# DCASE-REPO/DESED_task

Measured on AMD Instinct MI355X. Metric: 10s-clips/sec CRNN mean-teacher train @batch48, higher is better.
Workload: dtype f32 (fp32 storage and accumulation; the dense contractions of the wide layers run as split-bf16 MFMA, 3 bf16 products per fp32 product, fp32-level accuracy; everything else exact f32)

## Files before the change

### desed_task_amd/csrc/sed_common.h

```cpp
#pragma once

#ifdef SED_EMU
#include "hip_emu.h"
#else
#include <hip/hip_runtime.h>
#define SED_DYN_SMEM(name) extern __shared__ __attribute__((aligned(16))) char name[]
#define SED_LAUNCH(kern, grid, block, smem, stream, ...) \
    hipLaunchKernelGGL(kern, grid, block, smem, stream, __VA_ARGS__)
typedef float f32x16 __attribute__((ext_vector_type(16)));
typedef float f32x4 __attribute__((ext_vector_type(4)));
typedef short s16x8 __attribute__((ext_vector_type(8)));
#endif

#include <stdint.h>

#define SED_API extern "C" __attribute__((visibility("default")))

#define SED_MAX_SMEM(kern, bytes) \
    (void)hipFuncSetAttribute((const void*)(kern), hipFuncAttributeMaxDynamicSharedMemorySize, (int)(bytes))

__global__ __launch_bounds__(256) static void sed_zero4_kernel(float* p0, int n0, float* p1, int n1, float* p2, int n2, float* p3, int n3) {
    const int i = blockIdx.x * 256 + threadIdx.x;
    if (i < n0) p0[i] = 0.f;
    if (i < n1) p1[i] = 0.f;
    if (i < n2) p2[i] = 0.f;
    if (i < n3) p3[i] = 0.f;
}
static inline void sed_zero4(hipStream_t s, float* p0, int n0, float* p1, int n1, float* p2, int n2, float* p3, int n3) {
    int n = n0 > n1 ? n0 : n1;
    n = n > n2 ? n : n2;
    n = n > n3 ? n : n3;
    if (n <= 0) return;
    SED_LAUNCH(sed_zero4_kernel, dim3((n + 255) / 256), dim3(256), 0, s, p0, n0, p1, n1, p2, n2, p3, n3);
}

#define SED_OK 0
#define SED_ERR_ARG (-1)
#define SED_ERR_LAUNCH (-2)
#define SED_ERR_UNSUPPORTED (-3)

enum { SED_TUNE_GLU_GRID_CAP = 0, SED_TUNE_GLU_BWD128_SPLIT = 1, SED_TUNE_CONVB_CK = 2, SED_TUNE_CONVB_MP = 3, SED_TUNE_B0_NOCENTER = 4, SED_TUNE_GLU_FWD128 = 5, SED_TUNE_WGRAD_NARROW = 6, SED_TUNE_WGRAD_CAP = 7,
       SED_TUNE_ATTN_VALU = 8, SED_TUNE_WGRAD_WIDE = 9, SED_TUNE_GRU_LDS_KB = 10, SED_TUNE_MEL_TAPS_MEM = 11, SED_TUNE_CONVB_TPW = 12, SED_TUNE_MEL_WAVE = 13, SED_TUNE_GEMM_NTN = 14, SED_TUNE_LINEAR_TILES = 15, SED_TUNE_COUNT = 16 };
extern int sed_tuning[SED_TUNE_COUNT];

static inline int sed_check_launch() {
    hipError_t e = hipGetLastError();
    return e == hipSuccess ? SED_OK : SED_ERR_LAUNCH;
}

__device__ __forceinline__ f32x16 mfma32(float a, float b, f32x16 c) {
#ifdef SED_EMU
    return emu_mfma_32x32x2(a, b, c);
#else
    return __builtin_amdgcn_mfma_f32_32x32x2f32(a, b, c, 0, 0, 0);
#endif
}
__device__ __forceinline__ int mfma32_row(int r, int lane) { return (r & 3) + 8 * (r >> 2) + 4 * (lane >> 5); }

__device__ __forceinline__ f32x4 mfma16(float a, float b, f32x4 c) {
#ifdef SED_EMU
    return emu_mfma_16x16x4(a, b, c);
#else
    return __builtin_amdgcn_mfma_f32_16x16x4f32(a, b, c, 0, 0, 0);
#endif
}

__device__ __forceinline__ f32x16 mfma32_bf16(s16x8 a, s16x8 b, f32x16 c) {
#ifdef SED_EMU
    return emu_mfma_32x32x16_bf16(a, b, c);
#else
    typedef __bf16 bf16x8_t __attribute__((ext_vector_type(8)));
    return __builtin_amdgcn_mfma_f32_32x32x16_bf16(__builtin_bit_cast(bf16x8_t, a), __builtin_bit_cast(bf16x8_t, b), c, 0, 0, 0);
#endif
}
__device__ __forceinline__ f32x4 mfma16_bf16(s16x8 a, s16x8 b, f32x4 c) {
#ifdef SED_EMU
    return emu_mfma_16x16x32_bf16(a, b, c);
#else
    typedef __bf16 bf16x8_t __attribute__((ext_vector_type(8)));
    return __builtin_amdgcn_mfma_f32_16x16x32_bf16(__builtin_bit_cast(bf16x8_t, a), __builtin_bit_cast(bf16x8_t, b), c, 0, 0, 0);
#endif
}
__device__ __forceinline__ unsigned short f32_to_bf16(float x) {
    unsigned u = __float_as_uint(x);
    u += 0x7FFFu + ((u >> 16) & 1u);
    return (unsigned short)(u >> 16);
}
__device__ __forceinline__ float bf16_to_f32(unsigned short h) { return __uint_as_float(((unsigned)h) << 16); }
__device__ __forceinline__ void bf16_split(float x, unsigned short& hi, unsigned short& lo) {
    hi = f32_to_bf16(x);
    lo = f32_to_bf16(x - bf16_to_f32(hi));
}

__device__ __forceinline__ float sed_sadd(float a, float b) {
#ifdef SED_EMU
    return a + b;
#else
    float r;
    asm("v_add_f32 %0, %1, %2" : "=v"(r) : "v"(a), "v"(b));
    return r;
#endif
}

__device__ __forceinline__ float sed_sfma(float a, float b, float c) {
#ifdef SED_EMU
    return fmaf(a, b, c);
#else
    float r;
    asm("v_fma_f32 %0, %1, %2, %3" : "=v"(r) : "v"(a), "v"(b), "v"(c));
    return r;
#endif
}

__device__ __forceinline__ void sed_sched_fence() {
#ifndef SED_EMU
    __builtin_amdgcn_sched_barrier(0);
#endif
}

__device__ __forceinline__ unsigned sed_alignbit(unsigned hi, unsigned lo, unsigned shift) {
#ifdef SED_EMU
    return (unsigned)(((((unsigned long long)hi) << 32) | lo) >> shift);
#else
    return __builtin_amdgcn_alignbit(hi, lo, shift);
#endif
}

template <class T_>
__device__ __forceinline__ void sed_pin(T_& x) {
#ifndef SED_EMU
    asm volatile("" : "+v"(x));
#else
    (void)x;
#endif
}
__device__ __forceinline__ void sed_opaque(int& x) {
#ifndef SED_EMU
    asm volatile("" : "+v"(x));
#else
    (void)x;
#endif
}

__device__ __forceinline__ int sed_wave_uniform(int x) {
#ifdef SED_EMU
    return x;
#else
    return __builtin_amdgcn_readfirstlane(x);
#endif
}

__device__ __forceinline__ void sed_wave_sync() {
#ifdef SED_EMU
    emu_wave_sync();
#else
    __builtin_amdgcn_fence(__ATOMIC_ACQ_REL, "wavefront");
    __builtin_amdgcn_wave_barrier();
#endif
}

__device__ __forceinline__ void bf16_split2(float a, float b, unsigned& hi, unsigned& lo) {
#ifdef SED_EMU
    unsigned short h0, l0, h1, l1;
    bf16_split(a, h0, l0);
    bf16_split(b, h1, l1);
    hi = (unsigned)h0 | ((unsigned)h1 << 16);
    lo = (unsigned)l0 | ((unsigned)l1 << 16);
#else
    typedef float f32x2_t __attribute__((ext_vector_type(2)));
    typedef __bf16 bf16x2_t __attribute__((ext_vector_type(2)));
    const f32x2_t v = {a, b};
    hi = __builtin_bit_cast(unsigned, __builtin_convertvector(v, bf16x2_t));
    const f32x2_t hf = {__uint_as_float(hi << 16), __uint_as_float(hi & 0xFFFF0000u)};
    lo = __builtin_bit_cast(unsigned, __builtin_convertvector(v - hf, bf16x2_t));
#endif
}

__device__ __forceinline__ f32x16 f32x16_zero() {
    f32x16 z;
#pragma unroll
    for (int i = 0; i < 16; ++i) z[i] = 0.f;
    return z;
}

__device__ __forceinline__ float sed_quad_xor1(float v) {
#ifdef SED_EMU
    return __shfl_xor(v, 1);
#else
    return __builtin_bit_cast(float, __builtin_amdgcn_update_dpp(0, __builtin_bit_cast(int, v), 0xB1, 0xF, 0xF, true));
#endif
}
__device__ __forceinline__ float sed_quad_xor2(float v) {
#ifdef SED_EMU
    return __shfl_xor(v, 2);
#else
    return __builtin_bit_cast(float, __builtin_amdgcn_update_dpp(0, __builtin_bit_cast(int, v), 0x4E, 0xF, 0xF, true));
#endif
}
__device__ __forceinline__ float sed_row_ror4(float v) {
#ifdef SED_EMU
    return __shfl_xor(v, 4);
#else
    return __builtin_bit_cast(float, __builtin_amdgcn_update_dpp(0, __builtin_bit_cast(int, v), 0x124, 0xF, 0xF, true));
#endif
}
__device__ __forceinline__ float sed_row_ror8(float v) {
#ifdef SED_EMU
    return __shfl_xor(v, 8);
#else
    return __builtin_bit_cast(float, __builtin_amdgcn_update_dpp(0, __builtin_bit_cast(int, v), 0x128, 0xF, 0xF, true));
#endif
}
__device__ __forceinline__ float sed_row16_max(float v) {
    v = fmaxf(v, sed_quad_xor1(v)); v = fmaxf(v, sed_quad_xor2(v));
    v = fmaxf(v, sed_row_ror4(v)); v = fmaxf(v, sed_row_ror8(v));
    return v;
}
__device__ __forceinline__ float sed_row16_sum(float v) {
    v += sed_quad_xor1(v); v += sed_quad_xor2(v);
    v += sed_row_ror4(v); v += sed_row_ror8(v);
    return v;
}
__device__ __forceinline__ float sed_half_mirror(float v) {
#ifdef SED_EMU
    return __shfl_xor(v, 7);
#else
    return __builtin_bit_cast(float, __builtin_amdgcn_update_dpp(0, __builtin_bit_cast(int, v), 0x141, 0xF, 0xF, true));
#endif
}
__device__ __forceinline__ float sed_quad_sum(float v) {
    v += sed_quad_xor1(v);
    v += sed_quad_xor2(v);
    return v;
}

__device__ __forceinline__ float wave_sum(float v) {
#pragma unroll
    for (int m = 32; m >= 1; m >>= 1) v += __shfl_xor(v, m);
    return v;
}
__device__ __forceinline__ float wave_min(float v) {
#pragma unroll
    for (int m = 32; m >= 1; m >>= 1) v = fminf(v, __shfl_xor(v, m));
    return v;
}
__device__ __forceinline__ float wave_max(float v) {
#pragma unroll
    for (int m = 32; m >= 1; m >>= 1) v = fmaxf(v, __shfl_xor(v, m));
    return v;
}

__device__ __forceinline__ uint32_t sed_mix32(uint32_t x) {
    x ^= x >> 16; x *= 0x85EBCA6Bu;
    x ^= x >> 13; x *= 0xC2B2AE35u;
    x ^= x >> 16;
    return x;
}
__device__ __forceinline__ uint32_t sed_hash(uint32_t idx, uint32_t seed) {
#ifdef SED_HASH_V1
    return sed_mix32(idx * 0x9E3779B1u + seed);
#else
    uint32_t x = idx * 0x9E3779B1u + sed_mix32(seed);
    x ^= x >> 15;
    return x * 0x2C1B3C6Du;
#endif
}

__device__ __forceinline__ void sed_specaug_draw(int* __restrict__ bounds, int b, int n, int f_param, int n_freq, int t_param,
                                                 int n_time, uint32_t seed) {
    const int i = n == 1 ? 0 : b;
    const float inv = 1.0f / 16777216.0f;
    int f0 = 0, f1 = 0, t0 = 0, t1 = 0;
    if (f_param >= 1) {
        const float value = (float)(sed_hash(4u * i + 0u, seed) >> 8) * inv * (float)f_param;
        const float min_value = (float)(sed_hash(4u * i + 1u, seed) >> 8) * inv * ((float)n_freq - value);
        f0 = (int)min_value;
        f1 = f0 + (int)value;
    }
    if (t_param >= 1) {
        const float value = (float)(sed_hash(4u * i + 2u, seed) >> 8) * inv * (float)t_param;
        const float min_value = (float)(sed_hash(4u * i + 3u, seed) >> 8) * inv * ((float)n_time - value);
        t0 = (int)min_value;
        t1 = t0 + (int)value;
    }
    bounds[4 * b] = f0; bounds[4 * b + 1] = f1; bounds[4 * b + 2] = t0; bounds[4 * b + 3] = t1;
}
__device__ __forceinline__ bool sed_keep(uint32_t idx, uint32_t seed, uint32_t threshold24) {
    return (sed_hash(idx, seed) >> 8) >= threshold24;
}

__device__ __forceinline__ float sed_sigmoid(float x) { return 1.0f / (1.0f + expf(-x)); }
__device__ __forceinline__ float sed_tanh(float x) { return 1.0f - 2.0f / (expf(2.0f * x) + 1.0f); }

__device__ __forceinline__ float sed_fast_exp(float x) {
#ifdef SED_EMU
    return exp2f(x * 1.44269504088896341f);
#else
    return __builtin_amdgcn_exp2f(x * 1.44269504088896341f);
#endif
}
__device__ __forceinline__ float sed_fast_rcp(float x) {
#ifdef SED_EMU
    return 1.0f / x;
#else
    return __builtin_amdgcn_rcpf(x);
#endif
}
__device__ __forceinline__ float sed_fast_sigmoid(float x) { return sed_fast_rcp(1.0f + sed_fast_exp(-x)); }
__device__ __forceinline__ float sed_fast_tanh(float x) { return 1.0f - 2.0f * sed_fast_rcp(sed_fast_exp(2.0f * x) + 1.0f); }

__device__ __forceinline__ void sed_wave_prio_high() {
#if !defined(SED_EMU) && !defined(SED_NO_SETPRIO)
    __builtin_amdgcn_s_setprio(3);
#endif
}

__device__ __forceinline__ void sed_mfma_prio(int on) {
#if !defined(SED_EMU) && !defined(SED_NO_SETPRIO)
    if (on) __builtin_amdgcn_s_setprio(1); else __builtin_amdgcn_s_setprio(0);
#else
    (void)on;
#endif
}

__device__ __forceinline__ void sed_dma16(const void* gptr, void* lds_wave_base) {
#ifdef SED_EMU
    memcpy((char*)lds_wave_base + 16 * emu_lane(), gptr, 16);
// ... 84 lines not shown
```

### desed_task_amd/csrc/sed_glu.hip

```cpp
#include "sed_common.h"

#ifndef GLU_ABL
#define GLU_ABL 0
#endif

template <int C, int PT, int PF>
struct GluGeom {
    static constexpr int WIN = PT * PF;
    static constexpr int CP = C + 1;
    static constexpr int NT = C >= 32 ? C / 32 : 1;
};

template <int PT, int PF>
__device__ __forceinline__ bool row_pixel(int m, int o0, int NWC, int fsh, int& o, int& t, int& f) {
    constexpr int WIN = PT * PF;
    const int q = m % WIN;
    o = o0 + m / WIN;
    const int to = o >> fsh, fo = o & ((1 << fsh) - 1);
    t = to * PT + q / PF;
    f = fo * PF + q % PF;
    return o < NWC;
}

template <int C, int PT, int PF>
// ... 1374 lines not shown
        bf16_split2(c, d, hv.y, lv.y);
        const int off = ch * RT + 4 * (rq ^ (2 * ((ch >> 4) & 7)));
        *(uint2*)(xth + off) = hv;
        *(uint2*)(xtl + off) = lv;
    };
    auto xhat4 = [&](int j, float* out4) {
        const int rqd = 8 * wm + 2 * j + hi, off = n * RT + 4 * (rqd ^ (2 * ((n >> 4) & 7)));
        const uint2 hv = *(const uint2*)(xth + off), lv = *(const uint2*)(xtl + off);
        out4[0] = bf16_pair_sum((unsigned short)(hv.x & 0xFFFFu), (unsigned short)(lv.x & 0xFFFFu));
        out4[1] = bf16_pair_sum((unsigned short)(hv.x >> 16), (unsigned short)(lv.x >> 16));
        out4[2] = bf16_pair_sum((unsigned short)(hv.y & 0xFFFFu), (unsigned short)(lv.y & 0xFFFFu));
        out4[3] = bf16_pair_sum((unsigned short)(hv.y >> 16), (unsigned short)(lv.y >> 16));
    };
    const float gsc = 0.5f * dscale;
    float g8n[8];
    auto load_g8 = [&](int tile_) {
        const int rbase = tile_ * ROWS + 32 * wm + 4 * hi;
#pragma unroll
        for (int j = 0; j < 4; ++j)
#pragma unroll
            for (int h = 0; h < 2; ++h) {
                const int rr = rbase + 8 * j + 2 * h;
                g8n[2 * j + h] = gout[(size_t)((rr < R ? rr : R - 1) / 2) * C + n];
            }
    };
    int tile = blockIdx.x;
    if (tile < ntiles) { load_tile(tile); load_g8(tile); }
    for (; tile < ntiles; tile += gridDim.x) {
        const int row0 = tile * ROWS;
        sed_opaque(lo); sed_opaque(hi); sed_opaque(n); sed_opaque(cq); sed_opaque(rq);
        normalise(ld0, row0 + 4 * rq); normalise(ld1, row0 + 4 * rq + 1); normalise(ld2, row0 + 4 * rq + 2); normalise(ld3, row0 + 4 * rq + 3);
        __syncthreads();
        store_rm(ld0, 4 * rq); store_rm(ld1, 4 * rq + 1); store_rm(ld2, 4 * rq + 2); store_rm(ld3, 4 * rq + 3);
        store_tr(ld0.x, ld1.x, ld2.x, ld3.x, 4 * cq);
        store_tr(ld0.y, ld1.y, ld2.y, ld3.y, 4 * cq + 1);
        store_tr(ld0.z, ld1.z, ld2.z, ld3.z, 4 * cq + 2);
        store_tr(ld0.w, ld1.w, ld2.w, ld3.w, 4 * cq + 3);
        __syncthreads();
        if (tile + (int)gridDim.x < ntiles) load_tile(tile + gridDim.x);
        float g8[8];
#pragma unroll
        for (int u = 0; u < 8; ++u) g8[u] = g8n[u];
        load_g8(tile + (int)gridDim.x < ntiles ? tile + gridDim.x : tile);
        f32x16 acc = f32x16_zero();
        {
            const unsigned short* ap = xh + (32 * wm + lo) * RS + 8 * hi;
#pragma unroll
            for (int ks = 0; ks < KS; ++ks) {
                const s16x8 a_hi = *(const s16x8*)(ap + 16 * ks);
                const s16x8 a_lo = *(const s16x8*)(ap + ROWS * RS + 16 * ks);
                acc = mfma32_bf16(a_lo, b1h[ks], acc);
                acc = mfma32_bf16(a_hi, b1l[ks], acc);
                acc = mfma32_bf16(a_hi, b1h[ks], acc);
            }
        }
#pragma unroll
        for (int j = 0; j < 4; ++j) {
            float dv[4], xq[4];
            xhat4(j, xq);
#pragma unroll
            for (int q = 0; q < 4; ++q) {
                const int r = 4 * j + q, m = 32 * wm + 8 * j + 4 * hi + q;
                const uint32_t e_idx = (uint32_t)(row0 + m) * (uint32_t)C + (uint32_t)n;
                float dlin = 0.f, e = 0.f;
                if (row0 + m < R) {
                    const float xn = fmaf(xq[q], gn, bn);
                    const float sg = sed_fast_sigmoid(xn);
                    const float lin = acc[r] + biasp;
                    const float g = sed_keep(e_idx, seed, thr24) ? g8[2 * j + (q >> 1)] * gsc : 0.f;
                    dlin = g * sg;
                    e = g * lin * sg * (1.0f - sg);
                }
                unsigned short hh, ll;
                bf16_split(dlin, hh, ll);
                dh[m * RS + n] = hh;
                dl[m * RS + n] = ll;
                dv[q] = dlin;
                acc[r] = e;
                a_dbg += dlin;
            }
            uint2 hv, lv;
            bf16_split2(dv[0], dv[1], hv.x, lv.x);
            bf16_split2(dv[2], dv[3], hv.y, lv.y);
            const int rqd = 8 * wm + 2 * j + hi;
            const int off = n * RT + 4 * (rqd ^ (2 * ((n >> 4) & 7)));
            *(uint2*)(dth + off) = hv;
            *(uint2*)(dtl + off) = lv;
        }
        __syncthreads();
        {
            const unsigned short* ap = dh + (32 * wm + lo) * RS + 8 * hi;
#pragma unroll
            for (int ks = 0; ks < KS; ++ks) {
                const s16x8 a_hi = *(const s16x8*)(ap + 16 * ks);
                const s16x8 a_lo = *(const s16x8*)(ap + ROWS * RS + 16 * ks);
                acc = mfma32_bf16(a_lo, b2h[ks], acc);
                acc = mfma32_bf16(a_hi, b2l[ks], acc);
                acc = mfma32_bf16(a_hi, b2h[ks], acc);
            }
        }
#pragma unroll
        for (int j = 0; j < 4; ++j) {
            float xq[4];
            xhat4(j, xq);
#pragma unroll
            for (int q = 0; q < 4; ++q) {
                const int r = 4 * j + q, m = 32 * wm + 8 * j + 4 * hi + q;
                if (row0 + m < R) {
                    const float dxn = acc[r];
                    a_dgam = fmaf(dxn, xq[q], a_dgam);
                    a_dbet += dxn;
                    dz[(size_t)(row0 + m) * C + n] = dxn * gn;
                }
            }
        }
#pragma unroll
        for (int i = 0; i < TPW; ++i) {
            const int id = NT3 >= 8 ? w * TPW + i : w % NT3, mt = id / NT, ct = id % NT;
            const int ks0 = NT3 >= 8 ? 0 : (w / NT3) * KS3;
            const int rowa = mt * 32 + lo, rowb = ct * 32 + lo;
#pragma unroll
            for (int ks = 0; ks < KS3; ++ks) {
                const int oct = 2 * (ks0 + ks) + hi;
                const int offa = rowa * RT + 8 * (oct ^ ((rowa >> 4) & 7)), offb = rowb * RT + 8 * (oct ^ ((rowb >> 4) & 7));
                const s16x8 a_hi = *(const s16x8*)(dth + offa), a_lo = *(const s16x8*)(dtl + offa);
                const s16x8 b_hi = *(const s16x8*)(xth + offb), b_lo = *(const s16x8*)(xtl + offb);
                P[i] = mfma32_bf16(a_lo, b_hi, P[i]);
                P[i] = mfma32_bf16(a_hi, b_lo, P[i]);
                P[i] = mfma32_bf16(a_hi, b_hi, P[i]);
            }
        }
    }
    float* mine = part + (size_t)blockIdx.x * (KSPLIT * C * C + WM * 3 * C);
#pragma unroll
    for (int i = 0; i < TPW; ++i) {
        const int id = NT3 >= 8 ? w * TPW + i : w % NT3, mt = id / NT, ct = id % NT, c = ct * 32 + lo;
        float* dst = mine + (NT3 >= 8 ? 0 : w / NT3) * C * C;
#pragma unroll
        for (int r = 0; r < 16; ++r) dst[(mt * 32 + mfma32_row(r, lane)) * C + c] = P[i][r];
    }
    a_dbg += __shfl_xor(a_dbg, 32); a_dgam += __shfl_xor(a_dgam, 32); a_dbet += __shfl_xor(a_dbet, 32);
    if (hi == 0) {
        float* dst = mine + KSPLIT * C * C + wm * 3 * C;
        dst[n] = a_dbg; dst[C + n] = a_dgam; dst[2 * C + n] = a_dbet;
    }
}
__global__ __launch_bounds__(512) void glu128_bwd_c_kernel(const float* __restrict__ y, const float* __restrict__ stats,
                                                           const float* __restrict__ gamma, const float* __restrict__ beta,
                                                           const float* __restrict__ Wg, const float* __restrict__ bg,
                                                           const float* __restrict__ gout, float* __restrict__ dz,
                                                           float* __restrict__ part, int B, int T, int F, uint32_t seed,
                                                           uint32_t thr24, float dscale, const unsigned* __restrict__ seed_dev) {
    if (seed_dev) seed += *seed_dev;
    constexpr int C = 128, ROWS = 64, RS = C, RT = ROWS, WS = C + 8, KS = C / 32, RB = ROWS / 16, NB = C / 16, KS3 = ROWS / 32;
    SED_DYN_SMEM(smem);
    unsigned short* xh = (unsigned short*)smem;
    unsigned short* xl = xh + ROWS * RS;
    unsigned short* xth = xl + ROWS * RS;
    unsigned short* xtl = xth + C * RT;
    unsigned short* dh = xtl + C * RT;
    unsigned short* dl = dh + ROWS * RS;
    unsigned short* dth = dl + ROWS * RS;
    unsigned short* dtl = dth + C * RT;
    const int tid = threadIdx.x, lane = tid & 63, w = tid >> 6;
    int i16 = lane & 15, g = lane >> 4;
    int n = 16 * w + i16;
    const int R = B * T * F, ntiles = (R + ROWS - 1) / ROWS;
    auto rm_off = [](int m, int k) { return m * RS + ((((k >> 3) ^ (m & 15))) << 3) + (k & 7); };
    auto tr_off = [](int ch, int row) { return ch * RT + ((((row >> 3) ^ ((ch >> 1) & 7))) << 3) + (row & 7); };
    unsigned short* wh = xh;
    unsigned short* wl = xh + 64 * WS;

    s16x8 b1h[KS], b1l[KS], b2h[KS], b2l[KS];
    float biasp = bg[n];
#pragma unroll
    for (int p = 0; p < C / 64; ++p) {
#pragma unroll
        for (int fold = 0; fold < 2; ++fold) {
            __syncthreads();
            for (int i = tid; i < 64 * (C / 4); i += 512) {
                const int row = i / (C / 4), q = i - row * (C / 4);
                float4 val = *(const float4*)(Wg + (size_t)(p * 64 + row) * C + 4 * q);
                if (fold) { val.x *= gamma[4 * q]; val.y *= gamma[4 * q + 1]; val.z *= gamma[4 * q + 2]; val.w *= gamma[4 * q + 3]; }
                uint2 hv, lv;
                bf16_split2(val.x, val.y, hv.x, lv.x);
                bf16_split2(val.z, val.w, hv.y, lv.y);
                *(uint2*)(wh + row * WS + 4 * q) = hv;
                *(uint2*)(wl + row * WS + 4 * q) = lv;
            }
            __syncthreads();
            if (!fold) {
#pragma unroll
                for (int kk = 0; kk < 2; ++kk) {
                    s16x8 fh, fl;
#pragma unroll
                    for (int e = 0; e < 8; ++e) {
                        fh[e] = (short)wh[(32 * kk + 8 * g + e) * WS + n];
                        fl[e] = (short)wl[(32 * kk + 8 * g + e) * WS + n];
                    }
                    b2h[2 * p + kk] = fh; b2l[2 * p + kk] = fl;
                }
                if (w / 4 == p) {
                    const int rown = n - p * 64;
                    float part_b = 0.f;
                    for (int k = 32 * g; k < 32 * g + 32; ++k)
                        part_b = fmaf(beta[k], bf16_pair_sum(wh[rown * WS + k], wl[rown * WS + k]), part_b);
                    part_b += __shfl_xor(part_b, 16);
                    part_b += __shfl_xor(part_b, 32);
                    biasp += part_b;
                }
            } else if (w / 4 == p) {
#pragma unroll
                for (int ks = 0; ks < KS; ++ks) {
                    b1h[ks] = *(const s16x8*)(wh + (n - p * 64) * WS + 32 * ks + 8 * g);
                    b1l[ks] = *(const s16x8*)(wl + (n - p * 64) * WS + 32 * ks + 8 * g);
                }
            }
        }
    }
    const float gn = gamma[n], bn = beta[n];
    int cq = tid % (C / 4), rq = tid / (C / 4);

    f32x4 P[NB];
#pragma unroll
    for (int i = 0; i < NB; ++i) P[i] = f32x4{0.f, 0.f, 0.f, 0.f};
    float a_dbg = 0.f, a_dgam = 0.f, a_dbet = 0.f;

    float4 ld0, ld1, ld2, ld3;
    auto load_row = [&](int row) -> float4 {
        float4 val = make_float4(0.f, 0.f, 0.f, 0.f);
        if (row < R && !(GLU_ABL & 4)) val = *(const float4*)(y + (size_t)row * C + 4 * cq);
        return val;
    };
    auto load_tile = [&](int tile) {
        const int row = tile * ROWS + 4 * rq;
        if ((tile + 1) * ROWS <= R && !(GLU_ABL & 4)) {
            const float* src = y + (size_t)row * C + 4 * cq;
            ld0 = *(const float4*)src; ld1 = *(const float4*)(src + C); ld2 = *(const float4*)(src + 2 * C); ld3 = *(const float4*)(src + 3 * C);
        } else {
            ld0 = load_row(row); ld1 = load_row(row + 1); ld2 = load_row(row + 2); ld3 = load_row(row + 3);
        }
    };
    auto normalise = [&](int tile) {
        const float4 mu = *(const float4*)(stats + 4 * cq), is = *(const float4*)(stats + C + 4 * cq);
        const int row = tile * ROWS + 4 * rq;
        auto nrm = [&](float4& v, int r) {
            const float keep = r < R ? 1.0f : 0.0f;
            v.x = (v.x - mu.x) * is.x * keep; v.y = (v.y - mu.y) * is.y * keep;
            v.z = (v.z - mu.z) * is.z * keep; v.w = (v.w - mu.w) * is.w * keep;
        };
        nrm(ld0, row); nrm(ld1, row + 1); nrm(ld2, row + 2); nrm(ld3, row + 3);
    };
    auto store_rm = [&](const float4 val, int m) {
        uint2 hv, lv;
        bf16_split2(val.x, val.y, hv.x, lv.x);
        bf16_split2(val.z, val.w, hv.y, lv.y);
        *(uint2*)(xh + rm_off(m, 4 * cq)) = hv;
        *(uint2*)(xl + rm_off(m, 4 * cq)) = lv;
    };
    auto store_tr = [&](float a, float b, float c, float d, int ch) {
        uint2 hv, lv;
        bf16_split2(a, b, hv.x, lv.x);
        bf16_split2(c, d, hv.y, lv.y);
        const int off = tr_off(ch, 4 * rq);
        *(uint2*)(xth + off) = hv;
        *(uint2*)(xtl + off) = lv;
    };
    auto xhat4 = [&](int rb, float* out4) {
        const int off = tr_off(n, 16 * rb + 4 * g);
        const uint2 hv = *(const uint2*)(xth + off), lv = *(const uint2*)(xtl + off);
        out4[0] = bf16_pair_sum((unsigned short)(hv.x & 0xFFFFu), (unsigned short)(lv.x & 0xFFFFu));
        out4[1] = bf16_pair_sum((unsigned short)(hv.x >> 16), (unsigned short)(lv.x >> 16));
        out4[2] = bf16_pair_sum((unsigned short)(hv.y & 0xFFFFu), (unsigned short)(lv.y & 0xFFFFu));
        out4[3] = bf16_pair_sum((unsigned short)(hv.y >> 16), (unsigned short)(lv.y >> 16));
    };
    auto gemm_rows = [&](const unsigned short* ph, const s16x8* bh, const s16x8* bl, f32x4* acc) {
#pragma unroll
        for (int ks = 0; ks < KS; ++ks) {
            s16x8 ah[RB], al[RB];
#pragma unroll
            for (int rb = 0; rb < RB; ++rb) {
                const unsigned short* ap = ph + rm_off(16 * rb + i16, 32 * ks + 8 * g);
                ah[rb] = *(const s16x8*)ap;
                al[rb] = *(const s16x8*)(ap + ROWS * RS);
            }
#pragma unroll
            for (int rb = 0; rb < RB; ++rb) acc[rb] = mfma16_bf16(al[rb], bh[ks], acc[rb]);
#pragma unroll
            for (int rb = 0; rb < RB; ++rb) acc[rb] = mfma16_bf16(ah[rb], bl[ks], acc[rb]);
#pragma unroll
            for (int rb = 0; rb < RB; ++rb) acc[rb] = mfma16_bf16(ah[rb], bh[ks], acc[rb]);
            sed_sched_fence();
        }
    };
    int tile = blockIdx.x;
    float g8n[2 * RB];
    auto load_g8 = [&](int tile_) {
#pragma unroll
        for (int rb = 0; rb < RB; ++rb)
#pragma unroll
            for (int h = 0; h < 2; ++h) {
                const int rr = tile_ * ROWS + 16 * rb + 4 * g + 2 * h;
                g8n[2 * rb + h] = (GLU_ABL & 4) ? 1.0f : gout[(size_t)((rr < R ? rr : 0) / 2) * C + n];
            }
    };
    if (tile < ntiles) { load_tile(tile); load_g8(tile); }
    for (; tile < ntiles; tile += gridDim.x) {
        const int row0 = tile * ROWS;
        sed_opaque(i16); sed_opaque(g); sed_opaque(n); sed_opaque(cq); sed_opaque(rq);
        normalise(tile);
        __syncthreads();
        store_rm(ld0, 4 * rq); store_rm(ld1, 4 * rq + 1); store_rm(ld2, 4 * rq + 2); store_rm(ld3, 4 * rq + 3);
        store_tr(ld0.x, ld1.x, ld2.x, ld3.x, 4 * cq);
        store_tr(ld0.y, ld1.y, ld2.y, ld3.y, 4 * cq + 1);
        store_tr(ld0.z, ld1.z, ld2.z, ld3.z, 4 * cq + 2);
        store_tr(ld0.w, ld1.w, ld2.w, ld3.w, 4 * cq + 3);
        __syncthreads();
        float g8[2 * RB];
#pragma unroll
        for (int rb = 0; rb < RB; ++rb)
#pragma unroll
            for (int h = 0; h < 2; ++h) {
                const int rr = row0 + 16 * rb + 4 * g + 2 * h;
                g8[2 * rb + h] = rr < R ? g8n[2 * rb + h] * (0.5f * dscale) : 0.f;
            }
        load_g8(tile + (int)gridDim.x < ntiles ? tile + gridDim.x : tile);
        f32x4 acc[RB];
#pragma unroll
        for (int rb = 0; rb < RB; ++rb) acc[rb] = f32x4{0.f, 0.f, 0.f, 0.f};
        if (!(GLU_ABL & 1)) gemm_rows(xh, b1h, b1l, acc);
#pragma unroll
        for (int rb = 0; rb < RB; ++rb) {
            unsigned short hh[4], ll[4];
            float xq[4];
            xhat4(rb, xq);
#pragma unroll
            for (int r = 0; r < 4; ++r) {
                const int m = 16 * rb + 4 * g + r;
                const uint32_t e_idx = (uint32_t)(row0 + m) * (uint32_t)C + (uint32_t)n;
                const float xn = fmaf(xq[r], gn, bn);
                const float sg = (GLU_ABL & 2) ? xn : sed_fast_sigmoid(xn);
                const float lin = acc[rb][r] + biasp;
                const float gq = ((GLU_ABL & 2) || sed_keep(e_idx, seed, thr24)) ? g8[2 * rb + (r >> 1)] : 0.f;
                const float dlin = gq * sg;
                const float e = gq * lin * sg * (1.0f - sg);
                bf16_split(dlin, hh[r], ll[r]);
                dh[rm_off(m, n)] = hh[r];
                dl[rm_off(m, n)] = ll[r];
                acc[rb][r] = e;
                a_dbg += dlin;
            }
            uint2 hv, lv;
            hv.x = (unsigned)hh[0] | ((unsigned)hh[1] << 16); hv.y = (unsigned)hh[2] | ((unsigned)hh[3] << 16);
            lv.x = (unsigned)ll[0] | ((unsigned)ll[1] << 16); lv.y = (unsigned)ll[2] | ((unsigned)ll[3] << 16);
            const int off = tr_off(n, 16 * rb + 4 * g);
            *(uint2*)(dth + off) = hv;
            *(uint2*)(dtl + off) = lv;
        }
        __syncthreads();
        if (!(GLU_ABL & 1)) gemm_rows(dh, b2h, b2l, acc);
        const bool full = row0 + ROWS <= R;
#pragma unroll
        for (int rb = 0; rb < RB; ++rb) {
            float xq[4];
            xhat4(rb, xq);
#pragma unroll
            for (int r = 0; r < 4; ++r) {
                const int m = 16 * rb + 4 * g + r;
                const float dxn = acc[rb][r];
                a_dgam = fmaf(dxn, xq[r], a_dgam);
                a_dbet += dxn;
                if (!(GLU_ABL & 8) && (full || row0 + m < R)) dz[(size_t)(row0 + m) * C + n] = dxn * gn;
            }
        }
        if (tile + (int)gridDim.x < ntiles) load_tile(tile + gridDim.x);
        if (!(GLU_ABL & 1)) {
            const int rowa = 16 * w + i16;
            s16x8 ah3, al3;
#pragma unroll
            for (int st = 0; st < 2 * KS3; ++st) {
                const int ks = st >> 1, c0 = 4 * (st & 1);
                if ((st & 1) == 0) {
                    const int offa = tr_off(rowa, 32 * ks + 8 * g);
                    ah3 = *(const s16x8*)(dth + offa);
                    al3 = *(const s16x8*)(dtl + offa);
                }
                s16x8 bh3[4], bl3[4];
#pragma unroll
                for (int q = 0; q < 4; ++q) {
                    const int offb = tr_off(16 * (c0 + q) + i16, 32 * ks + 8 * g);
                    bh3[q] = *(const s16x8*)(xth + offb);
                    bl3[q] = *(const s16x8*)(xtl + offb);
                }
#pragma unroll
                for (int q = 0; q < 4; ++q) P[c0 + q] = mfma16_bf16(al3, bh3[q], P[c0 + q]);
#pragma unroll
                for (int q = 0; q < 4; ++q) P[c0 + q] = mfma16_bf16(ah3, bl3[q], P[c0 + q]);
#pragma unroll
                for (int q = 0; q < 4; ++q) P[c0 + q] = mfma16_bf16(ah3, bh3[q], P[c0 + q]);
                sed_sched_fence();
            }
        }
    }
    float* mine = part + (size_t)blockIdx.x * (C * C + 3 * C);
#pragma unroll
    for (int cb = 0; cb < NB; ++cb)
#pragma unroll
        for (int r = 0; r < 4; ++r) mine[(16 * w + 4 * g + r) * C + 16 * cb + i16] = P[cb][r];
    a_dbg += __shfl_xor(a_dbg, 16); a_dgam += __shfl_xor(a_dgam, 16); a_dbet += __shfl_xor(a_dbet, 16);
    a_dbg += __shfl_xor(a_dbg, 32); a_dgam += __shfl_xor(a_dgam, 32); a_dbet += __shfl_xor(a_dbet, 32);
    if (g == 0) {
        float* dst = mine + C * C;
        dst[n] = a_dbg; dst[C + n] = a_dgam; dst[2 * C + n] = a_dbet;
    }
}
#define GBR_THREADS 1024
#define GBR_GROUPS (GBR_THREADS / 16)
__global__ __launch_bounds__(GBR_THREADS) void glu_bwd_reduce_kernel(const float* __restrict__ part, float* __restrict__ dWg,
                                                             float* __restrict__ dbg, float* __restrict__ dgamma,
                                                             float* __restrict__ dbeta, int nblk, int C, int KS, int WMS,
                                                             const float* __restrict__ gamma, const float* __restrict__ beta, int fix) {
    __shared__ float4 red[GBR_GROUPS][16];
    __shared__ float sdb[GBR_THREADS / 64];
    const int tid = threadIdx.x, col = tid & 15, grp = tid >> 4, e = blockIdx.x * 64 + 4 * col;
    const int CC = C * C, PART = KS * CC + WMS * 3 * C;
    const bool isw = e < CC;
    const int nsl = isw ? KS : WMS, sstride = isw ? CC : 3 * C;
    const size_t off = isw ? (size_t)e : (size_t)KS * CC + (e - CC);
    float4 acc = make_float4(0.f, 0.f, 0.f, 0.f);
    if (e < CC + 3 * C) {
        const int total = nblk * nsl;
#pragma unroll 4
        for (int i = grp; i < total; i += GBR_GROUPS) {
            const int b = i / nsl, k = i - b * nsl;
            const float4 v = *(const float4*)(part + (size_t)b * PART + off + (size_t)k * sstride);
            acc.x += v.x; acc.y += v.y; acc.z += v.z; acc.w += v.w;
        }
    }
    const bool need_dbn = fix && blockIdx.x * 64 < CC;
    float sacc = 0.f;
    if (need_dbn) {
        const int nrow = (blockIdx.x * 64) / C;
#pragma unroll 2
        for (int i = tid; i < nblk * WMS; i += GBR_THREADS) {
            const int b = i / WMS, k = i - b * WMS;
            sacc += part[(size_t)b * PART + (size_t)KS * CC + k * 3 * C + nrow];
        }
    }
    float4 gq = make_float4(0.f, 0.f, 0.f, 0.f), bq = gq;
    if (fix && isw && grp == 0) {
        const int c = e % C;
        gq = make_float4(gamma[c], gamma[c + 1], gamma[c + 2], gamma[c + 3]);
        bq = make_float4(beta[c], beta[c + 1], beta[c + 2], beta[c + 3]);
    }
    red[grp][col] = acc;
    if (need_dbn) {
        sacc = wave_sum(sacc);
        if ((tid & 63) == 0) sdb[tid >> 6] = sacc;
    }
    __syncthreads();
    float dbn = 0.f;
    if (need_dbn) {
#pragma unroll
        for (int w = 0; w < GBR_THREADS / 64; ++w) dbn += sdb[w];
    }
    if (grp == 0 && e < CC + 3 * C) {
#pragma unroll 8
        for (int g = 1; g < GBR_GROUPS; ++g) { const float4 v = red[g][col]; acc.x += v.x; acc.y += v.y; acc.z += v.z; acc.w += v.w; }
        if (fix && isw) {
            acc.x = fmaf(gq.x, acc.x, bq.x * dbn); acc.y = fmaf(gq.y, acc.y, bq.y * dbn);
            acc.z = fmaf(gq.z, acc.z, bq.z * dbn); acc.w = fmaf(gq.w, acc.w, bq.w * dbn);
        }
        float* dst;
        if (isw) dst = dWg + e;
        else {
            const int j2 = e - CC, which = j2 / C;
            dst = (which == 0 ? dbg : which == 1 ? dgamma : dbeta) + (j2 - which * C);
        }
        *(float4*)dst = acc;
    }
}
template <int C, bool SPLIT>
static int launch_glu_wide_bwd(const float* y, const float* stats, const float* gamma, const float* beta, const float* Wg,
                               const float* bg, const float* gout, float* dz, float* dWg, float* dbg, float* dgamma, float* dbeta,
                               float* scratch, int B, int T, int F, uint32_t seed, uint32_t thr24, float dscale, const unsigned* seed_dev, hipStream_t s) {
    constexpr int ROWS = 32 * (8 / (C / 32)), WMS = 8 / (C / 32), KS = (C / 32) * (C / 32) >= 8 ? 1 : 8 / ((C / 32) * (C / 32));
    if (!scratch) return SED_ERR_ARG;
    constexpr int SMEM = SPLIT ? 8 * (ROWS * (C + 8) + C * (ROWS + 8)) : (2 * ROWS + (C > 64 ? C : 0)) * (C + 1) * 4;
    const int ntiles = (B * T * F + ROWS - 1) / ROWS;
    const int cap = glu_grid_cap(256);
    int grid = ntiles < cap ? ntiles : cap;
    if (grid < 1) { sed_zero4(s, dWg, C * C, dbg, C, dgamma, C, dbeta, C); return SED_OK; }
    if (SPLIT && C == 128 && sed_tuning[SED_TUNE_GLU_BWD128_SPLIT] != 1) {
        constexpr int SMEM_C = 8 * 64 * 128 * 2;
        SED_MAX_SMEM(glu128_bwd_c_kernel, SMEM_C);
        SED_LAUNCH(glu128_bwd_c_kernel, dim3(grid), dim3(512), SMEM_C, s, y, stats, gamma, beta, Wg, bg, gout, dz, scratch, B, T, F,
                   seed, thr24, dscale, seed_dev);
        SED_LAUNCH(glu_bwd_reduce_kernel, dim3((C * C + 3 * C + 63) / 64), dim3(GBR_THREADS), 0, s, scratch, dWg, dbg, dgamma, dbeta, grid, C, 1, 1,
                   gamma, beta, 1);
        return sed_check_launch();
    }
    if (SPLIT) {
        SED_MAX_SMEM((glu_wide_bwd_b_kernel<C>), SMEM);
        SED_LAUNCH((glu_wide_bwd_b_kernel<C>), dim3(grid), dim3(512), SMEM, s, y, stats, gamma, beta, Wg, bg, gout, dz, scratch, B, T, F,
                   seed, thr24, dscale, seed_dev);
    } else {
        SED_MAX_SMEM((glu_wide_bwd_kernel<C>), SMEM);
        SED_LAUNCH((glu_wide_bwd_kernel<C>), dim3(grid), dim3(512), SMEM, s, y, stats, gamma, beta, Wg, bg, gout, dz, scratch, B, T, F,
                   seed, thr24, dscale, seed_dev);
    }
    SED_LAUNCH(glu_bwd_reduce_kernel, dim3((C * C + 3 * C + 63) / 64), dim3(GBR_THREADS), 0, s, scratch, dWg, dbg, dgamma, dbeta, grid, C, KS, WMS,
               gamma, beta, SPLIT ? 1 : 0);
    return sed_check_launch();
}

SED_API long long sed_glu_bwd_scratch_floats(int B, int T, int F, int C, int PT, int PF) {
    (void)B; (void)T; (void)F;
    if (PT == 1 && PF == 2 && (C == 64 || C == 128)) {
        const int nt3 = (C / 32) * (C / 32), ks = nt3 >= 8 ? 1 : 8 / nt3, wms = 8 / (C / 32);
        return 256LL * (ks * C * C + wms * 3 * C);
    }
    if (PT == 2 && PF == 2 && (C == 16 || C == 32)) return 1024LL * (C * C + 3 * C);
    return 0;
}

SED_API int sed_glu_bwd(const float* y, const float* stats, const float* gamma, const float* beta, const float* Wg,
                           const float* bg, const float* gout, float* dz, float* dWg, float* dbg, float* dgamma, float* dbeta,
                           float* scratch, int B, int T, int F, int C, int PT, int PF, unsigned seed, unsigned thr24, float dscale,
                           const unsigned* seed_dev, int split_bf16, void* stream) {
    hipStream_t s = (hipStream_t)stream;
    if (F % PF != 0) return SED_ERR_UNSUPPORTED;
    if (PT == 1 && PF == 2) {
        if (C == 128 && split_bf16 && sed_tuning[SED_TUNE_GLU_BWD128_SPLIT] != 3)
            return launch_glu_wide_bwd<128, true>(y, stats, gamma, beta, Wg, bg, gout, dz, dWg, dbg, dgamma, dbeta, scratch, B, T, F, seed, thr24, dscale, seed_dev, s);
        if (C == 64 && split_bf16) return launch_glu_wide_bwd<64, true>(y, stats, gamma, beta, Wg, bg, gout, dz, dWg, dbg, dgamma, dbeta, scratch, B, T, F, seed, thr24, dscale, seed_dev, s);
        if (C == 128) return launch_glu_wide_bwd<128, false>(y, stats, gamma, beta, Wg, bg, gout, dz, dWg, dbg, dgamma, dbeta, scratch, B, T, F, seed, thr24, dscale, seed_dev, s);
        if (C == 64) return launch_glu_wide_bwd<64, false>(y, stats, gamma, beta, Wg, bg, gout, dz, dWg, dbg, dgamma, dbeta, scratch, B, T, F, seed, thr24, dscale, seed_dev, s);
    }
    const bool lds_free32 = C == 32 && PT == 2 && PF == 2 && F % 16 == 0 && T >= 2;
    if (T % PT != 0 && !lds_free32) {
        const int tail = T % PT, rowf4 = F * C / 4;
        const long long n4 = (long long)B * tail * rowf4;
        int grid = (int)((n4 + 255) / 256);
        if (grid > 2048) grid = 2048;
        SED_LAUNCH(glu_zero_tail_kernel, dim3(grid), dim3(256), 0, s, dz, n4, T, T - tail, tail * rowf4, (long long)T * rowf4);
    }
    if ((C == 16 && PT == 2 && PF == 2 && F % 8 == 0) || (C == 32 && PT == 2 && PF == 2 && F % 16 == 0)) {
        const int nrows = B * (T / 2);
        int grid = (nrows + 3) / 4;
        const int cap = C == 32 ? glu_grid_cap(512) : 1024;
        if (grid > cap) grid = cap;
        if (grid < 1) { sed_zero4(s, dWg, C * C, dbg, C, dgamma, C, dbeta, C); return SED_OK; }
        if (!scratch) return SED_ERR_ARG;
        if (C == 16)
            SED_LAUNCH(glu16_bwd_kernel, dim3(grid), dim3(256), 0, s, y, stats, gamma, beta, Wg, bg, gout, dz, scratch, B, T, F, seed, thr24,
                       dscale, seed_dev);
        else
            SED_LAUNCH(glu32_bwd_kernel, dim3(grid), dim3(256), 0, s, y, stats, gamma, beta, Wg, bg, gout, dz, scratch, B, T, F, seed, thr24,
                       dscale, seed_dev);
        SED_LAUNCH(glu_bwd_reduce_kernel, dim3((C * C + 3 * C + 63) / 64), dim3(GBR_THREADS), 0, s, scratch, dWg, dbg, dgamma, dbeta, grid, C, 1, 1,
                   gamma, beta, 0);
        return sed_check_launch();
    }
    sed_zero4(s, dWg, C * C, dbg, C, dgamma, C, dbeta, C);
#define GLU_CASE(c, pt, pf)                                                                                              \
    if (C == c && PT == pt && PF == pf)                                                                                  \
        return launch_glu_bwd<c, pt, pf>(y, stats, gamma, beta, Wg, bg, gout, dz, dWg, dbg, dgamma, dbeta, B, T, F, seed, thr24, \
                                         dscale, seed_dev, s);
    GLU_CASE(16, 2, 2) GLU_CASE(32, 2, 2)
#undef GLU_CASE
    return SED_ERR_UNSUPPORTED;
}

template <int C>
__global__ __launch_bounds__(256) void bn_bwd_apply_kernel(const float* __restrict__ y, float* __restrict__ dz,
                                                           const float* __restrict__ stats, const float* __restrict__ gamma,
                                                           const float* __restrict__ dgamma, const float* __restrict__ dbeta,
                                                           float* __restrict__ dbias, size_t npix, float inv_count, int training) {
    constexpr int V = C / 4, RPI = 256 / V;
    const int tid = threadIdx.x, v = tid % V, r0 = tid / V;
    float mean[4], istd[4], m1[4], m2[4];
#pragma unroll
    for (int i = 0; i < 4; ++i) {
        const int c = 4 * v + i;
        mean[i] = stats[c];
        istd[i] = stats[C + c];
        m1[i] = training ? gamma[c] * dbeta[c] * inv_count : 0.f;
        m2[i] = training ? gamma[c] * dgamma[c] * inv_count : 0.f;
    }
    if (blockIdx.x == 0 && tid < C) dbias[tid] = training ? 0.f : stats[C + tid] * gamma[tid] * dbeta[tid];
    for (size_t p = (size_t)blockIdx.x * RPI + r0; p < npix; p += (size_t)gridDim.x * RPI) {
        const float4 yv = *(const float4*)(y + p * C + 4 * v);
        float4 g = *(const float4*)(dz + p * C + 4 * v);
        g.x = istd[0] * (g.x - m1[0] - (yv.x - mean[0]) * istd[0] * m2[0]);
        g.y = istd[1] * (g.y - m1[1] - (yv.y - mean[1]) * istd[1] * m2[1]);
        g.z = istd[2] * (g.z - m1[2] - (yv.z - mean[2]) * istd[2] * m2[2]);
        g.w = istd[3] * (g.w - m1[3] - (yv.w - mean[3]) * istd[3] * m2[3]);
        *(float4*)(dz + p * C + 4 * v) = g;
    }
}
SED_API int sed_bn_bwd_apply(const float* y, float* dz, const float* stats, const float* gamma, const float* dgamma,
                                const float* dbeta, float* dbias, long long npix, int C, int training, void* stream) {
    hipStream_t s = (hipStream_t)stream;
    if (npix <= 0) return SED_OK;
    const float inv = 1.0f / (float)npix;
    int grid = (int)((npix * (C / 4) + 255) / 256);
    if (grid > 4096) grid = 4096;
#define BN_CASE(c) \
    if (C == c) { SED_LAUNCH((bn_bwd_apply_kernel<c>), dim3(grid), dim3(256), 0, s, y, dz, stats, gamma, dgamma, dbeta, dbias, (size_t)npix, inv, training); return sed_check_launch(); }
    BN_CASE(16) BN_CASE(32) BN_CASE(64) BN_CASE(128)
#undef BN_CASE
    return SED_ERR_UNSUPPORTED;
}
```

Baseline: 16050.

## Double-buffer GLU128 backward tiles and use LDS transpose reads instead of transposed copies

```diff
diff --git a/desed_task_amd/csrc/sed_common.h b/desed_task_amd/csrc/sed_common.h
--- a/desed_task_amd/csrc/sed_common.h
+++ b/desed_task_amd/csrc/sed_common.h
@@ -173,6 +173,21 @@
     hi = __builtin_bit_cast(unsigned, __builtin_convertvector(v, bf16x2_t));
     const f32x2_t hf = {__uint_as_float(hi << 16), __uint_as_float(hi & 0xFFFF0000u)};
     lo = __builtin_bit_cast(unsigned, __builtin_convertvector(v - hf, bf16x2_t));
+#endif
+}
+
+template <class OFF>
+__device__ __forceinline__ uint2 sed_lds_read_tr16(const unsigned short* img, OFF off, int r0, int c0, int lane) {
+#ifdef SED_EMU
+    const int col = c0 + (lane & 15);
+    uint2 v;
+    v.x = (unsigned)img[off(r0, col)] | ((unsigned)img[off(r0 + 1, col)] << 16);
+    v.y = (unsigned)img[off(r0 + 2, col)] | ((unsigned)img[off(r0 + 3, col)] << 16);
+    return v;
+#else
+    typedef short s16x4_t __attribute__((ext_vector_type(4)));
+    const unsigned short* p = img + off(r0 + ((lane >> 2) & 3), c0 + 4 * (lane & 3));
+    return __builtin_bit_cast(uint2, __builtin_amdgcn_ds_read_tr16_b64_v4i16((__attribute__((address_space(3))) s16x4_t*)p));
 #endif
 }
 
diff --git a/desed_task_amd/csrc/sed_glu.hip b/desed_task_amd/csrc/sed_glu.hip
--- a/desed_task_amd/csrc/sed_glu.hip
+++ b/desed_task_amd/csrc/sed_glu.hip
@@ -1550,35 +1550,40 @@
                                                            float* __restrict__ part, int B, int T, int F, uint32_t seed,
                                                            uint32_t thr24, float dscale, const unsigned* __restrict__ seed_dev) {
     if (seed_dev) seed += *seed_dev;
-    constexpr int C = 128, ROWS = 64, RS = C, RT = ROWS, WS = C + 8, KS = C / 32, RB = ROWS / 16, NB = C / 16, KS3 = ROWS / 32;
+    constexpr int C = 128, ROWS = 64, WS = C + 8, KS = C / 32, RB = ROWS / 16, NB = C / 16, KS3 = ROWS / 32, PL = ROWS * C;
     SED_DYN_SMEM(smem);
-    unsigned short* xh = (unsigned short*)smem;
-    unsigned short* xl = xh + ROWS * RS;
-    unsigned short* xth = xl + ROWS * RS;
-    unsigned short* xtl = xth + C * RT;
-    unsigned short* dh = xtl + C * RT;
-    unsigned short* dl = dh + ROWS * RS;
-    unsigned short* dth = dl + ROWS * RS;
-    unsigned short* dtl = dth + C * RT;
-    const int tid = threadIdx.x, lane = tid & 63, w = tid >> 6;
-    int i16 = lane & 15, g = lane >> 4;
+    unsigned short* xbuf = (unsigned short*)smem;
+    unsigned short* dth = xbuf + 4 * PL;
+    unsigned short* dtl = dth + PL;
+    const int tid = threadIdx.x, w = tid >> 6;
+    int lane = tid & 63, i16 = lane & 15, g = lane >> 4;
     int n = 16 * w + i16;
     const int R = B * T * F, ntiles = (R + ROWS - 1) / ROWS;
-    auto rm_off = [](int m, int k) { return m * RS + ((((k >> 3) ^ (m & 15))) << 3) + (k & 7); };
-    auto tr_off = [](int ch, int row) { return ch * RT + ((((row >> 3) ^ ((ch >> 1) & 7))) << 3) + (row & 7); };
-    unsigned short* wh = xh;
-    unsigned short* wl = xh + 64 * WS;
+    auto x_off = [](int m, int k) {
+        return m * C + ((((k >> 3) ^ (int)(0xEC13B9468A75DF20ull >> (4 * (m & 15)))) & 15) << 3) + (k & 7);
+    };
+    auto d_off = [](int ch, int row) {
+        return ch * ROWS + ((((row >> 3) ^ (int)(0x4307256152163470ull >> (4 * ((ch & 3) | ((ch >> 1) & 12))))) & 7) << 3) + (row & 7);
+    };
+    unsigned short* wh = xbuf;
+    unsigned short* wl = xbuf + C * WS;
 
     s16x8 b1h[KS], b1l[KS], b2h[KS], b2l[KS];
     float biasp = bg[n];
-#pragma unroll
-    for (int p = 0; p < C / 64; ++p) {
+    {
+        float4 wv[C * (C / 4) / 512];
+#pragma unroll
+        for (int j = 0; j < C * (C / 4) / 512; ++j) {
+            const int i = tid + 512 * j, row = i / (C / 4), q = i - row * (C / 4);
+            wv[j] = *(const float4*)(Wg + (size_t)row * C + 4 * q);
+        }
 #pragma unroll
         for (int fold = 0; fold < 2; ++fold) {
-            __syncthreads();
-            for (int i = tid; i < 64 * (C / 4); i += 512) {
-                const int row = i / (C / 4), q = i - row * (C / 4);
-                float4 val = *(const float4*)(Wg + (size_t)(p * 64 + row) * C + 4 * q);
+            if (fold) __syncthreads();
+#pragma unroll
+            for (int j = 0; j < C * (C / 4) / 512; ++j) {
+                const int i = tid + 512 * j, row = i / (C / 4), q = i - row * (C / 4);
+                float4 val = wv[j];
                 if (fold) { val.x *= gamma[4 * q]; val.y *= gamma[4 * q + 1]; val.z *= gamma[4 * q + 2]; val.w *= gamma[4 * q + 3]; }
                 uint2 hv, lv;
                 bf16_split2(val.x, val.y, hv.x, lv.x);
@@ -1589,29 +1594,26 @@
             __syncthreads();
             if (!fold) {
 #pragma unroll
-                for (int kk = 0; kk < 2; ++kk) {
+                for (int ks = 0; ks < KS; ++ks) {
                     s16x8 fh, fl;
 #pragma unroll
                     for (int e = 0; e < 8; ++e) {
-                        fh[e] = (short)wh[(32 * kk + 8 * g + e) * WS + n];
-                        fl[e] = (short)wl[(32 * kk + 8 * g + e) * WS + n];
+                        fh[e] = (short)wh[(32 * ks + 8 * g + e) * WS + n];
+                        fl[e] = (short)wl[(32 * ks + 8 * g + e) * WS + n];
                     }
-                    b2h[2 * p + kk] = fh; b2l[2 * p + kk] = fl;
+                    b2h[ks] = fh; b2l[ks] = fl;
                 }
-                if (w / 4 == p) {
-                    const int rown = n - p * 64;
-                    float part_b = 0.f;
-                    for (int k = 32 * g; k < 32 * g + 32; ++k)
-                        part_b = fmaf(beta[k], bf16_pair_sum(wh[rown * WS + k], wl[rown * WS + k]), part_b);
-                    part_b += __shfl_xor(part_b, 16);
-                    part_b += __shfl_xor(part_b, 32);
-                    biasp += part_b;
-                }
-            } else if (w / 4 == p) {
+                float part_b = 0.f;
+                for (int k = 32 * g; k < 32 * g + 32; ++k)
+                    part_b = fmaf(beta[k], bf16_pair_sum(wh[n * WS + k], wl[n * WS + k]), part_b);
+                part_b += __shfl_xor(part_b, 16);
+                part_b += __shfl_xor(part_b, 32);
+                biasp += part_b;
+            } else {
 #pragma unroll
                 for (int ks = 0; ks < KS; ++ks) {
-                    b1h[ks] = *(const s16x8*)(wh + (n - p * 64) * WS + 32 * ks + 8 * g);
-                    b1l[ks] = *(const s16x8*)(wl + (n - p * 64) * WS + 32 * ks + 8 * g);
+                    b1h[ks] = *(const s16x8*)(wh + n * WS + 32 * ks + 8 * g);
+                    b1l[ks] = *(const s16x8*)(wl + n * WS + 32 * ks + 8 * g);
                 }
             }
         }
@@ -1624,7 +1626,7 @@
     for (int i = 0; i < NB; ++i) P[i] = f32x4{0.f, 0.f, 0.f, 0.f};
     float a_dbg = 0.f, a_dgam = 0.f, a_dbet = 0.f;
 
-    float4 ld0, ld1, ld2, ld3;
+    float4 ld0 = make_float4(0.f, 0.f, 0.f, 0.f), ld1 = ld0, ld2 = ld0, ld3 = ld0;
     auto load_row = [&](int row) -> float4 {
         float4 val = make_float4(0.f, 0.f, 0.f, 0.f);
         if (row < R && !(GLU_ABL & 4)) val = *(const float4*)(y + (size_t)row * C + 4 * cq);
@@ -1649,47 +1651,32 @@
         };
         nrm(ld0, row); nrm(ld1, row + 1); nrm(ld2, row + 2); nrm(ld3, row + 3);
     };
-    auto store_rm = [&](const float4 val, int m) {
+    auto store_row = [&](unsigned short* xb, const float4 val, int m) {
         uint2 hv, lv;
         bf16_split2(val.x, val.y, hv.x, lv.x);
         bf16_split2(val.z, val.w, hv.y, lv.y);
-        *(uint2*)(xh + rm_off(m, 4 * cq)) = hv;
-        *(uint2*)(xl + rm_off(m, 4 * cq)) = lv;
-    };
-    auto store_tr = [&](float a, float b, float c, float d, int ch) {
-        uint2 hv, lv;
-        bf16_split2(a, b, hv.x, lv.x);
-        bf16_split2(c, d, hv.y, lv.y);
-        const int off = tr_off(ch, 4 * rq);
-        *(uint2*)(xth + off) = hv;
-        *(uint2*)(xtl + off) = lv;
-    };
-    auto xhat4 = [&](int rb, float* out4) {
-        const int off = tr_off(n, 16 * rb + 4 * g);
-        const uint2 hv = *(const uint2*)(xth + off), lv = *(const uint2*)(xtl + off);
+        *(uint2*)(xb + x_off(m, 4 * cq)) = hv;
+        *(uint2*)(xb + PL + x_off(m, 4 * cq)) = lv;
+    };
+    auto xhat4 = [&](const unsigned short* xb, int rb, float* out4) {
+        const uint2 hv = sed_lds_read_tr16(xb, x_off, 16 * rb + 4 * g, 16 * w, lane);
+        const uint2 lv = sed_lds_read_tr16(xb + PL, x_off, 16 * rb + 4 * g, 16 * w, lane);
         out4[0] = bf16_pair_sum((unsigned short)(hv.x & 0xFFFFu), (unsigned short)(lv.x & 0xFFFFu));
         out4[1] = bf16_pair_sum((unsigned short)(hv.x >> 16), (unsigned short)(lv.x >> 16));
         out4[2] = bf16_pair_sum((unsigned short)(hv.y & 0xFFFFu), (unsigned short)(lv.y & 0xFFFFu));
         out4[3] = bf16_pair_sum((unsigned short)(hv.y >> 16), (unsigned short)(lv.y >> 16));
     };
-    auto gemm_rows = [&](const unsigned short* ph, const s16x8* bh, const s16x8* bl, f32x4* acc) {
-#pragma unroll
-        for (int ks = 0; ks < KS; ++ks) {
-            s16x8 ah[RB], al[RB];
-#pragma unroll
-            for (int rb = 0; rb < RB; ++rb) {
-                const unsigned short* ap = ph + rm_off(16 * rb + i16, 32 * ks + 8 * g);
-                ah[rb] = *(const s16x8*)ap;
-                al[rb] = *(const s16x8*)(ap + ROWS * RS);
-            }
-#pragma unroll
-            for (int rb = 0; rb < RB; ++rb) acc[rb] = mfma16_bf16(al[rb], bh[ks], acc[rb]);
-#pragma unroll
-            for (int rb = 0; rb < RB; ++rb) acc[rb] = mfma16_bf16(ah[rb], bl[ks], acc[rb]);
-#pragma unroll
-            for (int rb = 0; rb < RB; ++rb) acc[rb] = mfma16_bf16(ah[rb], bh[ks], acc[rb]);
-            sed_sched_fence();
-        }
+    auto frag8 = [](const uint2 a, const uint2 b) {
+        const uint4 v = make_uint4(a.x, a.y, b.x, b.y);
+        return __builtin_bit_cast(s16x8, v);
+    };
+    auto mfma_step = [&](const s16x8* ah, const s16x8* al, const s16x8 bh, const s16x8 bl, f32x4* acc) {
+#pragma unroll
+        for (int rb = 0; rb < RB; ++rb) acc[rb] = mfma16_bf16(al[rb], bh, acc[rb]);
+#pragma unroll
+        for (int rb = 0; rb < RB; ++rb) acc[rb] = mfma16_bf16(ah[rb], bl, acc[rb]);
+#pragma unroll
+        for (int rb = 0; rb < RB; ++rb) acc[rb] = mfma16_bf16(ah[rb], bh, acc[rb]);
     };
     int tile = blockIdx.x;
     float g8n[2 * RB];
@@ -1703,17 +1690,18 @@
             }
     };
     if (tile < ntiles) { load_tile(tile); load_g8(tile); }
-    for (; tile < ntiles; tile += gridDim.x) {
+    __syncthreads();
+    if (tile < ntiles) {
+        normalise(tile);
+        store_row(xbuf, ld0, 4 * rq); store_row(xbuf, ld1, 4 * rq + 1); store_row(xbuf, ld2, 4 * rq + 2); store_row(xbuf, ld3, 4 * rq + 3);
+        if (tile + (int)gridDim.x < ntiles) load_tile(tile + gridDim.x);
+    }
+    __syncthreads();
+    for (int buf = 0; tile < ntiles; tile += gridDim.x, buf ^= 1) {
         const int row0 = tile * ROWS;
-        sed_opaque(i16); sed_opaque(g); sed_opaque(n); sed_opaque(cq); sed_opaque(rq);
-        normalise(tile);
-        __syncthreads();
-        store_rm(ld0, 4 * rq); store_rm(ld1, 4 * rq + 1); store_rm(ld2, 4 * rq + 2); store_rm(ld3, 4 * rq + 3);
-        store_tr(ld0.x, ld1.x, ld2.x, ld3.x, 4 * cq);
-        store_tr(ld0.y, ld1.y, ld2.y, ld3.y, 4 * cq + 1);
-        store_tr(ld0.z, ld1.z, ld2.z, ld3.z, 4 * cq + 2);
-        store_tr(ld0.w, ld1.w, ld2.w, ld3.w, 4 * cq + 3);
-        __syncthreads();
+        sed_opaque(lane); sed_opaque(i16); sed_opaque(g); sed_opaque(n); sed_opaque(cq); sed_opaque(rq);
+        const unsigned short* xc = xbuf + buf * 2 * PL;
+        unsigned short* xnx = xbuf + (buf ^ 1) * 2 * PL;
         float g8[2 * RB];
 #pragma unroll
         for (int rb = 0; rb < RB; ++rb)
@@ -1726,12 +1714,25 @@
         f32x4 acc[RB];
 #pragma unroll
         for (int rb = 0; rb < RB; ++rb) acc[rb] = f32x4{0.f, 0.f, 0.f, 0.f};
-        if (!(GLU_ABL & 1)) gemm_rows(xh, b1h, b1l, acc);
+        if (!(GLU_ABL & 1)) {
+#pragma unroll
+            for (int ks = 0; ks < KS; ++ks) {
+                s16x8 ah[RB], al[RB];
+#pragma unroll
+                for (int rb = 0; rb < RB; ++rb) {
+                    const unsigned short* ap = xc + x_off(16 * rb + i16, 32 * ks + 8 * g);
+                    ah[rb] = *(const s16x8*)ap;
+                    al[rb] = *(const s16x8*)(ap + PL);
+                }
+                mfma_step(ah, al, b1h[ks], b1l[ks], acc);
+                sed_sched_fence();
+            }
+        }
 #pragma unroll
         for (int rb = 0; rb < RB; ++rb) {
             unsigned short hh[4], ll[4];
             float xq[4];
-            xhat4(rb, xq);
+            xhat4(xc, rb, xq);
 #pragma unroll
             for (int r = 0; r < 4; ++r) {
                 const int m = 16 * rb + 4 * g + r;
@@ -1743,25 +1744,41 @@
                 const float dlin = gq * sg;
                 const float e = gq * lin * sg * (1.0f - sg);
                 bf16_split(dlin, hh[r], ll[r]);
-                dh[rm_off(m, n)] = hh[r];
-                dl[rm_off(m, n)] = ll[r];
                 acc[rb][r] = e;
                 a_dbg += dlin;
             }
             uint2 hv, lv;
             hv.x = (unsigned)hh[0] | ((unsigned)hh[1] << 16); hv.y = (unsigned)hh[2] | ((unsigned)hh[3] << 16);
             lv.x = (unsigned)ll[0] | ((unsigned)ll[1] << 16); lv.y = (unsigned)ll[2] | ((unsigned)ll[3] << 16);
-            const int off = tr_off(n, 16 * rb + 4 * g);
+            const int off = d_off(n, 16 * rb + 4 * g);
             *(uint2*)(dth + off) = hv;
             *(uint2*)(dtl + off) = lv;
         }
-        __syncthreads();
-        if (!(GLU_ABL & 1)) gemm_rows(dh, b2h, b2l, acc);
+        if (!(GLU_ABL & 64)) __syncthreads();
+        normalise(tile + (int)gridDim.x);
+#pragma unroll
+        for (int ks = 0; ks < KS; ++ks) {
+            s16x8 ah[RB], al[RB];
+            int ln = lane;
+            sed_opaque(ln);
+            const int ch0 = 32 * ks + 8 * (ln >> 4);
+            if (!(GLU_ABL & 1)) {
+#pragma unroll
+                for (int rb = 0; rb < RB; ++rb) {
+                    ah[rb] = frag8(sed_lds_read_tr16(dth, d_off, ch0, 16 * rb, ln), sed_lds_read_tr16(dth, d_off, ch0 + 4, 16 * rb, ln));
+                    al[rb] = frag8(sed_lds_read_tr16(dtl, d_off, ch0, 16 * rb, ln), sed_lds_read_tr16(dtl, d_off, ch0 + 4, 16 * rb, ln));
+                }
+            }
+            store_row(xnx, ks == 0 ? ld0 : ks == 1 ? ld1 : ks == 2 ? ld2 : ld3, 4 * rq + ks);
+            if (!(GLU_ABL & 1)) mfma_step(ah, al, b2h[ks], b2l[ks], acc);
+            sed_sched_fence();
+        }
+        if (tile + 2 * (int)gridDim.x < ntiles) load_tile(tile + 2 * gridDim.x);
         const bool full = row0 + ROWS <= R;
 #pragma unroll
         for (int rb = 0; rb < RB; ++rb) {
             float xq[4];
-            xhat4(rb, xq);
+            xhat4(xc, rb, xq);
 #pragma unroll
             for (int r = 0; r < 4; ++r) {
                 const int m = 16 * rb + 4 * g + r;
@@ -1771,24 +1788,24 @@
                 if (!(GLU_ABL & 8) && (full || row0 + m < R)) dz[(size_t)(row0 + m) * C + n] = dxn * gn;
             }
         }
-        if (tile + (int)gridDim.x < ntiles) load_tile(tile + gridDim.x);
         if (!(GLU_ABL & 1)) {
-            const int rowa = 16 * w + i16;
             s16x8 ah3, al3;
 #pragma unroll
             for (int st = 0; st < 2 * KS3; ++st) {
-                const int ks = st >> 1, c0 = 4 * (st & 1);
+                int ln = lane;
+                sed_opaque(ln);
+                const int ks = st >> 1, c0 = 4 * (st & 1), k0 = 32 * ks + 8 * (ln >> 4);
                 if ((st & 1) == 0) {
-                    const int offa = tr_off(rowa, 32 * ks + 8 * g);
+                    const int offa = d_off(16 * w + (ln & 15), k0);
                     ah3 = *(const s16x8*)(dth + offa);
                     al3 = *(const s16x8*)(dtl + offa);
                 }
                 s16x8 bh3[4], bl3[4];
 #pragma unroll
                 for (int q = 0; q < 4; ++q) {
-                    const int offb = tr_off(16 * (c0 + q) + i16, 32 * ks + 8 * g);
-                    bh3[q] = *(const s16x8*)(xth + offb);
-                    bl3[q] = *(const s16x8*)(xtl + offb);
+                    const int cb = 16 * (c0 + q);
+                    bh3[q] = frag8(sed_lds_read_tr16(xc, x_off, k0, cb, ln), sed_lds_read_tr16(xc, x_off, k0 + 4, cb, ln));
+                    bl3[q] = frag8(sed_lds_read_tr16(xc + PL, x_off, k0, cb, ln), sed_lds_read_tr16(xc + PL, x_off, k0 + 4, cb, ln));
                 }
 #pragma unroll
                 for (int q = 0; q < 4; ++q) P[c0 + q] = mfma16_bf16(al3, bh3[q], P[c0 + q]);
@@ -1799,6 +1816,7 @@
                 sed_sched_fence();
             }
         }
+        if (!(GLU_ABL & 64)) __syncthreads();
     }
     float* mine = part + (size_t)blockIdx.x * (C * C + 3 * C);
 #pragma unroll
@@ -1890,7 +1908,7 @@
     int grid = ntiles < cap ? ntiles : cap;
     if (grid < 1) { sed_zero4(s, dWg, C * C, dbg, C, dgamma, C, dbeta, C); return SED_OK; }
     if (SPLIT && C == 128 && sed_tuning[SED_TUNE_GLU_BWD128_SPLIT] != 1) {
-        constexpr int SMEM_C = 8 * 64 * 128 * 2;
+        constexpr int SMEM_C = 6 * 64 * 128 * 2;
         SED_MAX_SMEM(glu128_bwd_c_kernel, SMEM_C);
         SED_LAUNCH(glu128_bwd_c_kernel, dim3(grid), dim3(512), SMEM_C, s, y, stats, gamma, beta, Wg, bg, gout, dz, scratch, B, T, F,
                    seed, thr24, dscale, seed_dev);
```

Result: no change. 15930 (-0.8%).
